# zongh5a/MDF-Net

Hardware: AMD Instinct MI355X
Metric: views/sec at DTU 1600x1200x5-view x4-scale (higher is better)
Workload: dtype f32; 1 GPU; DTU eval 1600x1184 (1600x1200 cropped as load/dtueval.py:34), 5 views, 3 cost-volume stages + x2 refine = 4 output scales, hypotheses (48,24,8), batch 1 per rank, seeded random weights (pth/dtu_29.pth is not available offline); parallelism=views sharded over 1 rank(s), no collective

## Files before the change

### mdf-net_amd/csrc/wino2d.hip

```cpp
#include <cstdlib>
#include <type_traits>
#include "common.h"
#include "conv_lds_common.h"
#define W3_PINNED_TILES_32
#include "wino3d_acc.h"

namespace {

template <int I, int N, typename F>
__device__ __forceinline__ void static_for(F&& f) {
  if constexpr (I < N) {
    f(std::integral_constant<int, I>{});
    static_for<I + 1, N>(f);
  }
}

struct Wino2dParams {
  const float* x;
  const float* wpack;
  const float* alpha;
  const float* beta;
  const float* res;
  float* y;
  float res_scale;
  int B, H, W, relu;
  int tiles_h, tiles_w, n_tiles;
};

template <int CIN, int COUT>
struct W2 {
  static_assert(CIN % 16 == 0 && COUT % 16 == 0 && COUT <= 64, "2-D Winograd form: Cin, Cout multiples of 16, Cout <= 64");
  static constexpr int NCH = CIN / 16, NT = COUT / 16, NG = CIN / 4;
  static constexpr int WN = (CIN >= 64) ? 2 : 1, NTW = NT / WN, WM = 4 / WN;
  static_assert(NT % WN == 0 && NTW >= 1 && NTW <= 2, "cout tiles per wave");
  static constexpr int TH = 2 * WM, TWO = 32;
  static constexpr int PH = TH + 2, PW = TWO + 2;
  static constexpr int NPP = PH * PW;
  static constexpr int S = round_s(NPP, 4, 2);
  static constexpr int PLANE = CIN * S;
  static constexpr int RING = 3;
  static constexpr int NPOS = NG * NPP;
  static constexpr int NFILL = (NPOS + 255) / 256;
  static constexpr int EPI_OFF = RING * PLANE;
  static constexpr int FRAG = 64 * 4;
  static constexpr int NSTEP = NCH * 16;
  static constexpr bool WL = ((size_t)(RING * PLANE + 128 + NSTEP * NT * FRAG) * sizeof(float) <= 160 * 1024);
  static constexpr int W_OFF = EPI_OFF + 128;
  static constexpr size_t LDS_BYTES = (size_t)(RING * PLANE + 128 + (WL ? NSTEP * NT * FRAG : 0)) * sizeof(float);
  static_assert(S > NPP, "a pad vector per group takes the fill's surplus lanes");
};

#ifndef MDF_W2_DIAG
#define MDF_W2_DIAG 0
#endif
#ifndef MDF_W2_HOLD_REL
#define MDF_W2_HOLD_REL 0
#endif
#ifndef MDF_W2_NA
#define MDF_W2_NA 4
#endif
#ifndef MDF_W2_WRITE_AB
#define MDF_W2_WRITE_AB 2
#endif

template <int CIN, int COUT, int NA, int WRITE_AB, bool S2D>
__global__ __launch_bounds__(256, 1) void wino2d_kernel(const Wino2dParams p) {
  typedef W2<CIN, COUT> C;
  constexpr int NCH = C::NCH, NT = C::NT, S = C::S, PW = C::PW, NPP = C::NPP, NFILL = C::NFILL, NSTEP = C::NSTEP;
  constexpr int AH = NA - 1;
  static_assert(NSTEP % NA == 0, "the fragment ring must close over a tile");
  extern __shared__ __attribute__((aligned(16))) float lds[];

  const int tid = threadIdx.x, lane = tid & 63;
  const int wave = __builtin_amdgcn_readfirstlane(tid >> 6);
  const int q = lane >> 4, n16 = lane & 15;
  const __amdgpu_buffer_rsrc_t wres = make_rsrc(p.wpack, (unsigned)(NSTEP * NT * 64 * 4 * 4));
  const int wvoff = lane * 16;
  const int wm = wave / C::WN, wn = wave % C::WN;
  constexpr int NTW = C::NTW;
  const int lane_lds = (q * S + wm * 2 * PW + n16 * 2) * 4;

  if (tid < 128) {
    const int c = tid & 63;
    lds[C::EPI_OFF + tid] = (tid < 64) ? ((c < COUT && p.alpha) ? p.alpha[c] : 1.f) : ((c < COUT && p.beta) ? p.beta[c] : 0.f);
  }
  if constexpr (C::WL) {
    constexpr int NV = NSTEP * NT * 64;
    for (int v = tid; v < NV; v += 256)
      *reinterpret_cast<float4*>(lds + C::W_OFF + v * 4) = *reinterpret_cast<const float4*>(p.wpack + (size_t)v * 4);
  }

  constexpr bool HOLD_REL = (NFILL <= 11) || (NTW == 1) || MDF_W2_HOLD_REL;
  constexpr int CM = S2D ? CIN / 4 : CIN;
  [[maybe_unused]] constexpr int GPP = CM / 4;
  auto rel_of = [&](int row, int col, int g) -> int {
    if constexpr (S2D) {
      const int par = g / GPP, c4 = g - par * GPP;
      return (((2 * row + (par >> 1)) * (2 * p.W) + 2 * col + (par & 1)) * CM + c4 * 4) * 4;
    } else {
      return ((row * p.W + col) * CIN + g * 4) * 4;
    }
  };
  int f_lds[NFILL], f_rc[NFILL], f_rel[HOLD_REL ? NFILL : 1];
#pragma unroll
  for (int k = 0; k < NFILL; ++k) {
    const int idx = tid + k * 256;
    const int glo = idx & 3, r = idx >> 2;
    const int v = r % NPP, g = (r / NPP) * 4 + glo;
    const bool live = idx < C::NPOS;
    const int row = live ? v / PW : 0x40, col = v % PW;
    f_lds[k] = live ? (g * S + v) * 4 : NPP * 4;
    f_rc[k] = (row << 16) | (col << 8) | g;
    if constexpr (HOLD_REL) f_rel[k] = live ? rel_of(row, col, g) : (int)0x80000000u;
  }

  const unsigned lb = mdf::xcd_remap(blockIdx.x, gridDim.x);
  const int t_begin = __builtin_amdgcn_readfirstlane((int)((unsigned long long)lb * (unsigned)p.n_tiles / gridDim.x));
  const int t_end = __builtin_amdgcn_readfirstlane((int)((unsigned long long)(lb + 1) * (unsigned)p.n_tiles / gridDim.x));
  if (t_begin >= t_end) return;

  float4 pf[NFILL];
  struct TileAt { int b, th, tw; };
  auto tile_at = [&](int t) -> TileAt {
    const int tw = t % p.tiles_w, rest = t / p.tiles_w;
    return TileAt{__builtin_amdgcn_readfirstlane(rest / p.tiles_h), __builtin_amdgcn_readfirstlane(rest % p.tiles_h), __builtin_amdgcn_readfirstlane(tw)};
  };
  auto tile_advance = [&](TileAt& c) {
    if (++c.tw == p.tiles_w) {
      c.tw = 0;
      if (++c.th == p.tiles_h) { c.th = 0; ++c.b; }
    }
  };
  auto issue_tile = [&](const TileAt& at, bool valid) {
    const int b = valid ? at.b : 0, h0 = (valid ? at.th : 0) * C::TH, w0 = (valid ? at.tw : 0) * C::TWO;
    const long long org = S2D ? ((long long)b * (2 * p.H) + 2 * (h0 - 1)) * (2 * p.W) + 2 * (w0 - 1)
                              : ((long long)b * p.H + (h0 - 1)) * p.W + (w0 - 1);
    const float* pz = p.x + org * CM;
    const unsigned long long pa = (unsigned long long)pz;
    const unsigned lo = (unsigned)__builtin_amdgcn_readfirstlane((int)(unsigned)pa), hi = (unsigned)__builtin_amdgcn_readfirstlane((int)(unsigned)(pa >> 32));
    const unsigned nrec = (!valid || (MDF_W2_DIAG & 1)) ? 0u : 0x7fffffffu;
    const __amdgpu_buffer_rsrc_t xr = make_rsrc((const void*)(((unsigned long long)hi << 32) | lo), nrec);
    const int r_lo = 1 - h0, r_hi = p.H + 1 - h0, c_lo = 1 - w0, c_hi = p.W + 1 - w0;
    if constexpr (HOLD_REL) {
      if (r_lo <= 0 && r_hi >= C::PH && c_lo <= 0 && c_hi >= C::PW) {
#pragma unroll
        for (int k = 0; k < NFILL; ++k) {
          const u32x4_t v = __builtin_amdgcn_raw_buffer_load_b128(xr, f_rel[k], 0, 0);
          pf[k] = make_float4(__uint_as_float(v.x), __uint_as_float(v.y), __uint_as_float(v.z), __uint_as_float(v.w));
        }
        return;
      }
    }
#pragma unroll
    for (int k = 0; k < NFILL; ++k) {
      const int row = f_rc[k] >> 16, col = (f_rc[k] >> 8) & 0xff;
      const bool ok = row >= r_lo && row < r_hi && col >= c_lo && col < c_hi;
      int rel;
      if constexpr (HOLD_REL) rel = f_rel[k];
      else rel = rel_of(row, col, f_rc[k] & 0xff);
      const u32x4_t v = __builtin_amdgcn_raw_buffer_load_b128(xr, ok ? rel : (int)0x80000000u, 0, 0);
      pf[k] = make_float4(__uint_as_float(v.x), __uint_as_float(v.y), __uint_as_float(v.z), __uint_as_float(v.w));
    }
  };
  auto write_tile = [&](int slot) {
#pragma unroll
    for (int k = 0; k < NFILL; ++k) *reinterpret_cast<float4*>(lds + slot * C::PLANE + f_lds[k]) = pf[k];
  };

  f32x2_t V[16][2], Dn[16][2];
  auto read_elem = [&](int slot, int ch, int e) {
    const int i = e >> 2, j = e & 3;
    float t[4];
    lds_frag<4>(lds + slot * C::PLANE + lane_lds + ((ch * 4) * S + i * PW + j) * 4, t);
    Dn[e][0] = (f32x2_t){t[0], t[1]};
    Dn[e][1] = (f32x2_t){t[2], t[3]};
  };
  auto transform = [&]() {
#pragma unroll
    for (int j = 0; j < 4; ++j)
#pragma unroll
      for (int c = 0; c < 2; ++c) {
        const f32x2_t d0 = Dn[j][c], d1 = Dn[4 + j][c], d2 = Dn[8 + j][c], d3 = Dn[12 + j][c];
        Dn[j][c] = d0 - d2; Dn[4 + j][c] = d1 + d2; Dn[8 + j][c] = d2 - d1; Dn[12 + j][c] = d1 - d3;
      }
#pragma unroll
    for (int a = 0; a < 4; ++a)
#pragma unroll
      for (int c = 0; c < 2; ++c) {
        const f32x2_t e0 = Dn[a * 4][c], e1 = Dn[a * 4 + 1][c], e2 = Dn[a * 4 + 2][c], e3 = Dn[a * 4 + 3][c];
        V[a * 4][c] = e0 - e2; V[a * 4 + 1][c] = e1 + e2; V[a * 4 + 2][c] = e2 - e1; V[a * 4 + 3][c] = e1 - e3;
      }
#pragma unroll
    for (int e = 0; e < 16; ++e)
#pragma unroll
      for (int c = 0; c < 2; ++c) asm volatile("" : "+v"(V[e][c]));
  };

  float af[NA][NTW][4];
  auto load_a = [&](int i, int buf) {
#pragma unroll
    for (int ntl = 0; ntl < NTW; ++ntl) {
      if constexpr (C::WL) lds_frag<4>(lds + C::W_OFF + (i * NT + wn * NTW + ntl) * C::FRAG + lane * 4, af[buf][ntl]);
      else buf_load_to<4>(wres, wvoff, (i * NT + wn * NTW + ntl) * (64 * 4 * 4), af[buf][ntl]);
    }
  };

  auto epilogue = [&](const TileAt& at) {
    const int b = at.b, h0 = at.th * C::TH, w0 = at.tw * C::TWO;
    if (h0 + 2 * wm >= p.H) return;
    const float* epi_tab = lds + C::EPI_OFF;
    asm volatile("s_nop 15\n\ts_nop 15" ::: "memory");
    static_for<0, NTW>([&](auto ntc) {
      constexpr int nt = decltype(ntc)::value;
      const int c0 = (wn * NTW + nt) * 16 + 4 * q;
      float yv[2][2][4];
      static_for<0, 2>([&](auto k2c) {
        constexpr int k2 = decltype(k2c)::value;
        float m[16][2];
        static_for<0, 16>([&](auto abc) { AccTile<nt * 16 + decltype(abc)::value>::template read2<k2>(m[decltype(abc)::value]); });
        f32x2_t srow[2][4];
#pragma unroll
        for (int bb = 0; bb < 4; ++bb) {
          const f32x2_t m0 = {m[bb][0], m[bb][1]}, m1 = {m[4 + bb][0], m[4 + bb][1]};
          const f32x2_t m2 = {m[8 + bb][0], m[8 + bb][1]}, m3 = {m[12 + bb][0], m[12 + bb][1]};
          srow[0][bb] = m0 + m1 + m2;
          srow[1][bb] = m1 - m2 - m3;
        }
#pragma unroll
        for (int pr = 0; pr < 2; ++pr) {
          const f32x2_t y0 = srow[pr][0] + srow[pr][1] + srow[pr][2];
          const f32x2_t y1 = srow[pr][1] - srow[pr][2] - srow[pr][3];
          yv[pr][0][2 * k2] = y0[0]; yv[pr][0][2 * k2 + 1] = y0[1];
          yv[pr][1][2 * k2] = y1[0]; yv[pr][1][2 * k2 + 1] = y1[1];
        }
      });
      float al_l[4], be_l[4];
#pragma unroll
      for (int k = 0; k < 4; ++k) { al_l[k] = epi_tab[c0 + k]; be_l[k] = epi_tab[64 + c0 + k]; }
#pragma unroll
      for (int pr = 0; pr < 2; ++pr) {
        const int h = h0 + 2 * wm + pr;
        if (h >= p.H) continue;
        const size_t row_vox = ((size_t)b * p.H + h) * p.W;
#pragma unroll
        for (int rr = 0; rr < 2; ++rr) {
          const int ow = w0 + 2 * n16 + rr;
          if (ow >= p.W) continue;
          float ov[4];
#pragma unroll
          for (int k = 0; k < 4; ++k) {
            ov[k] = yv[pr][rr][k] * al_l[k] + be_l[k];
            if (p.relu) ov[k] = fmaxf(ov[k], 0.f);
          }
          const size_t oi = (row_vox + ow) * COUT + c0;
          if (p.res) {
            const float4 rv = *reinterpret_cast<const float4*>(p.res + oi);
            ov[0] = rv.x + ov[0] * p.res_scale; ov[1] = rv.y + ov[1] * p.res_scale;
            ov[2] = rv.z + ov[2] * p.res_scale; ov[3] = rv.w + ov[3] * p.res_scale;
          }
          if (!(MDF_W2_DIAG & 2) || ov[0] == 1234.5f) *reinterpret_cast<float4*>(p.y + oi) = make_float4(ov[0], ov[1], ov[2], ov[3]);
        }
      }
    });
  };

  auto step = [&](auto rc, const TileAt& at, const TileAt& at_next2, bool valid_next2, bool has_next) {
    constexpr int R = decltype(rc)::value;
    constexpr int SLOT_N = (R + 1) % 3;
    static_for<0, NSTEP>([&](auto ic) {
      constexpr int i = decltype(ic)::value;
      constexpr int ch = i / 16, ab = i % 16;
      constexpr bool last_chunk = (ch == NCH - 1);
      if (!(MDF_W2_DIAG & 16)) load_a((i + AH) % NSTEP, (i + AH) % NA);
      if constexpr (ch == 0 && ab == WRITE_AB) {
        if (has_next) {
          write_tile(SLOT_N);
          __syncthreads();
        }
      }
      if constexpr (ab > WRITE_AB && ab <= WRITE_AB + 8 && !(MDF_W2_DIAG & 32)) {
        constexpr int e0 = 2 * (ab - WRITE_AB - 1);
        if constexpr (!last_chunk) { read_elem(R, ch + 1, e0); read_elem(R, ch + 1, e0 + 1); }
        else { read_elem(SLOT_N, 0, e0); read_elem(SLOT_N, 0, e0 + 1); }
      }
      __builtin_amdgcn_sched_barrier(0);
      static_for<0, NTW>([&](auto ntc) {
        constexpr int nt = decltype(ntc)::value;
        constexpr int T = nt * 16 + ab;
        if constexpr (ch == 0) AccTile<T>::mfma_fresh(af[i % NA][nt][0], V[ab][0][0]);
        else AccTile<T>::mfma(af[i % NA][nt][0], V[ab][0][0]);
        AccTile<T>::mfma(af[i % NA][nt][1], V[ab][0][1]);
        AccTile<T>::mfma(af[i % NA][nt][2], V[ab][1][0]);
        AccTile<T>::mfma(af[i % NA][nt][3], V[ab][1][1]);
      });
      __builtin_amdgcn_sched_barrier(0);
      if constexpr (ab == 15 && !last_chunk) { if (!(MDF_W2_DIAG & 8)) transform(); }
    });
    issue_tile(at_next2, valid_next2);
    if (!(MDF_W2_DIAG & 8)) transform();
    if (!(MDF_W2_DIAG & 4)) epilogue(at);
  };

  int t = t_begin;
  const int t_last = t_end - 1;
  TileAt at = tile_at(t), at2 = at;
  issue_tile(at, true);
  write_tile(0);
  __syncthreads();
  tile_advance(at2);
  issue_tile(at2, t < t_last);
  tile_advance(at2);
#pragma unroll
  for (int e = 0; e < 16; ++e) read_elem(0, 0, e);
  transform();
#pragma unroll
  for (int i = 0; i < AH; ++i) load_a(i, i % NA);

#define W2_STEP(RR)                                                                        \
  {                                                                                        \
    const bool has_next = t < t_last;                                                      \
    step(std::integral_constant<int, RR>{}, at, at2, t + 2 <= t_last, has_next);           \
    if (!has_next) break;                                                                  \
    ++t; tile_advance(at); tile_advance(at2);                                              \
  }
  for (;;) {
    W2_STEP(0)
    W2_STEP(1)
    W2_STEP(2)
  }
#undef W2_STEP
}

template <int CIN, int COUT, bool S2D = false>
int launch_wino2d(Wino2dParams& p, hipStream_t st) {
  typedef W2<CIN, COUT> C;
  constexpr int NA = MDF_W2_NA, WRITE_AB = MDF_W2_WRITE_AB;
  p.tiles_h = (p.H + C::TH - 1) / C::TH;
  p.tiles_w = (p.W + C::TWO - 1) / C::TWO;
  const long long tiles = (long long)p.B * p.tiles_h * p.tiles_w;
  if (tiles >= (1ll << 31)) return MDF_EUNSUPPORTED;
  p.n_tiles = (int)tiles;
  auto kern = &wino2d_kernel<CIN, COUT, NA, WRITE_AB, S2D>;
  static bool attr_done_dev[64] = {};
  int dev_id = 0;
  (void)hipGetDevice(&dev_id);
  bool& attr_done = attr_done_dev[(dev_id >= 0 && dev_id < 64) ? dev_id : 0];
  if (!attr_done || dev_id >= 64) {
    hipError_t e = hipFuncSetAttribute(reinterpret_cast<const void*>(kern), hipFuncAttributeMaxDynamicSharedMemorySize, (int)C::LDS_BYTES);
    if (e != hipSuccess) return mdf::fail(MDF_EHIP, "hipFuncSetAttribute(dynamic LDS %zu): %s", (size_t)C::LDS_BYTES, hipGetErrorString(e));
    attr_done = true;
  }
  long long grid = 256;
  if (const char* g = getenv("MDF_WINO2D_GRID")) { if (atoi(g) > 0) grid = atoi(g); }
  if (grid > tiles / 2) grid = tiles / 2;
  if (grid < 1) grid = 1;
  hipLaunchKernelGGL(kern, dim3((unsigned)grid), dim3(256), C::LDS_BYTES, st, p);
  return mdf::check_launch("wino2d_kernel");
}

}

int mdf_wino2d_dispatch(const float* x, const float* wpack_wino, const float* alpha, const float* beta, const float* res, float res_scale,
                        float* y, int B, int H, int W, int Cin, int Cout, int relu, void* stream) {
  Wino2dParams p{};
  p.x = x; p.wpack = wpack_wino; p.alpha = alpha; p.beta = beta; p.res = res; p.res_scale = res_scale; p.y = y;
  p.B = B; p.H = H; p.W = W; p.relu = relu;
  if ((long long)B * H * W * Cin * 4 >= (1ll << 31)) return MDF_EUNSUPPORTED;
  if (Cin == 16 && Cout == 16 && getenv("MDF_WINO2D_16")) return launch_wino2d<16, 16>(p, (hipStream_t)stream);
  if (Cin == 32 && Cout == 32) return launch_wino2d<32, 32>(p, (hipStream_t)stream);
  if (Cin == 64 && Cout == 64) return launch_wino2d<64, 64>(p, (hipStream_t)stream);
  return MDF_EUNSUPPORTED;
}

int mdf_wino2d_s2d_dispatch(const float* x, const float* wpack_k5w, const float* alpha, const float* beta, float* y, int B, int Ho, int Wo,
                            int Cin_mem, int Cout, int relu, void* stream) {
  Wino2dParams p{};
  p.x = x; p.wpack = wpack_k5w; p.alpha = alpha; p.beta = beta; p.res = nullptr; p.res_scale = 0.f; p.y = y;
  p.B = B; p.H = Ho; p.W = Wo; p.relu = relu;
  if ((long long)B * Ho * Wo * 4 * Cin_mem * 4 >= (1ll << 31)) return MDF_EUNSUPPORTED;
  if (Cin_mem == 16 && Cout == 32) return launch_wino2d<64, 32, true>(p, (hipStream_t)stream);
  if (Cin_mem == 8 && Cout == 16) return launch_wino2d<32, 16, true>(p, (hipStream_t)stream);
  return MDF_EUNSUPPORTED;
}
```

### mdf-net_amd/csrc/wino3d.hip

```cpp
#include <cstdlib>
#include <type_traits>
#include "common.h"
#include "conv_lds_common.h"
#include "wino3d_acc.h"

namespace {

template <int I, int N, typename F>
__device__ __forceinline__ void static_for(F&& f) {
  if constexpr (I < N) {
    f(std::integral_constant<int, I>{});
    static_for<I + 1, N>(f);
  }
}

struct Wino3dParams {
  const float* x;
  const float* wpack;
  const float* alpha;
  const float* beta;
  const float* res;
  float* y;
  float res_scale;
  int B, D, H, W, relu;
  int tiles_h, tiles_w;
  long long total;
};

template <int CIN, int COUT>
struct W3 {
  static_assert(CIN % 16 == 0 && COUT % 16 == 0 && COUT <= 64, "Winograd 3-D form: Cin, Cout multiples of 16");
  static constexpr int NCH = CIN / 16, NT = COUT / 16, NG = CIN / 4;
  static constexpr int WM = 4 / NT;
  static constexpr int TH = 2 * WM, TWO = 32;
  static constexpr int PH = TH + 2, PW = TWO + 2;
  static constexpr int NPP = PH * PW;
  static constexpr int S = round_s(NPP, 4, 2);
  static constexpr int PLANE = CIN * S;
  static constexpr int RING = 3;
  static constexpr int NPOS = NG * NPP;
  static constexpr int NFILL = (NPOS + 255) / 256;
  static constexpr int EPI_OFF = RING * PLANE;
  static constexpr int FRAG = 64 * 4;
  static constexpr int WL = ((size_t)(RING * PLANE + 128 + 3 * NCH * 16 * NT * FRAG) * sizeof(float) <= 160 * 1024) ? 3 : 0;
  static constexpr int W_OFF = EPI_OFF + 128;
  static constexpr size_t LDS_BYTES = (size_t)(RING * PLANE + 128 + WL * NCH * 16 * NT * FRAG) * sizeof(float);
  static_assert(S > NPP, "a pad vector per group takes the fill's surplus lanes");
};

#ifndef MDF_W3_DIAG
#define MDF_W3_DIAG 0
#endif
#ifndef MDF_W3_NOMASK
#define MDF_W3_NOMASK 0
#endif
#ifndef MDF_W3_PF_AT_START
#define MDF_W3_PF_AT_START 0
#endif
#ifndef MDF_W3_NA
#define MDF_W3_NA 4
#endif
#ifndef MDF_W3_WRITE_AB
#define MDF_W3_WRITE_AB 2
#endif
template <int CIN, int COUT, int NA, int WRITE_AB>
__global__ __launch_bounds__(256, 1) void wino3d_kernel(const Wino3dParams p) {
  typedef W3<CIN, COUT> C;
  constexpr int NCH = C::NCH, NT = C::NT, S = C::S, PW = C::PW, NPP = C::NPP, NFILL = C::NFILL;
  constexpr int AH = NA - 1;
  constexpr int NSTEP = NCH * 16;
  static_assert(NSTEP % NA == 0, "the fragment ring must close over a plane");
  extern __shared__ __attribute__((aligned(16))) float lds[];

  const int tid = threadIdx.x, lane = tid & 63;
  const int wave = __builtin_amdgcn_readfirstlane(tid >> 6);
  const int q = lane >> 4, n16 = lane & 15;
  const int wm = wave / NT, wn = wave % NT;
  const __amdgpu_buffer_rsrc_t wres = make_rsrc(p.wpack, (unsigned)(3 * NCH * 16 * NT * 64 * 4 * 4));
  const int wvoff = lane * 16;
  const int lane_lds = (q * S + wm * 2 * PW + n16 * 2) * 4;

  if (tid < 128) {
    const int c = tid & 63;
    lds[C::EPI_OFF + tid] = (tid < 64) ? ((c < COUT && p.alpha) ? p.alpha[c] : 1.f) : ((c < COUT && p.beta) ? p.beta[c] : 0.f);
  }

  if constexpr (C::WL > 0) {
    constexpr int NV = C::WL * NSTEP * NT * 64;
    for (int v = tid; v < NV; v += 256)
      *reinterpret_cast<float4*>(lds + C::W_OFF + v * 4) = *reinterpret_cast<const float4*>(p.wpack + (size_t)v * 4);
  }

  int f_lds[NFILL];
#pragma unroll
  for (int k = 0; k < NFILL; ++k) {
    const int idx = tid + k * 256;
    const int glo = idx & 3, r = idx >> 2;
    const int v = r % NPP, ghi = r / NPP;
    f_lds[k] = (idx < C::NPOS) ? ((ghi * 4 + glo) * S + v) * 4 : NPP * 4;
  }

  const size_t plane_elems = (size_t)p.H * p.W * CIN;
  const unsigned plane_bytes = (unsigned)(plane_elems * 4);

  const unsigned lb = mdf::xcd_remap(blockIdx.x, gridDim.x);
  unsigned s_cur = (unsigned)((unsigned long long)lb * (unsigned)p.total / gridDim.x);
  const unsigned s_end = (unsigned)((unsigned long long)(lb + 1) * (unsigned)p.total / gridDim.x);

  while (s_cur < s_end) {
    const int tile_l = __builtin_amdgcn_readfirstlane((int)(s_cur / (unsigned)p.D));
    const int da = __builtin_amdgcn_readfirstlane((int)(s_cur - (unsigned)tile_l * (unsigned)p.D));
    const int db = __builtin_amdgcn_readfirstlane((int)min((unsigned)p.D, (unsigned)da + (s_end - s_cur)));
    s_cur += db - da;
    const int tw = __builtin_amdgcn_readfirstlane(tile_l % p.tiles_w);
    const int th = __builtin_amdgcn_readfirstlane((tile_l / p.tiles_w) % p.tiles_h);
    const int b = __builtin_amdgcn_readfirstlane(tile_l / (p.tiles_w * p.tiles_h));
    const int h0 = th * C::TH, w0 = tw * C::TWO;
    const bool wave_live = (h0 + 2 * wm) < p.H;

    unsigned f_off[NFILL];
    {
      int tid_l = tid;
      asm volatile("" : "+v"(tid_l));
#pragma unroll
      for (int k = 0; k < NFILL; ++k) {
        const int idx = tid_l + k * 256;
        const int glo = idx & 3, r2 = idx >> 2;
        const int v = r2 % NPP, g = (r2 / NPP) * 4 + glo;
        const int ih = h0 - 1 + v / PW, iw = w0 - 1 + v % PW;
        const bool ok = idx < C::NPOS && ih >= 0 && ih < p.H && iw >= 0 && iw < p.W;
        f_off[k] = ok ? (unsigned)(((ih * p.W + iw) * CIN + g * 4) * 4) : 0x80000000u;
      }
    }
    const float* xb = p.x + (size_t)b * p.D * plane_elems;
    float4 pf[NFILL];
    auto issue_plane = [&](int z) {
      const bool in = z >= 0 && z < p.D;
      const float* pz = xb + (size_t)(in ? z : 0) * plane_elems;
      const unsigned long long pa = (unsigned long long)pz;
      const unsigned lo = (unsigned)__builtin_amdgcn_readfirstlane((int)(unsigned)pa), hi = (unsigned)__builtin_amdgcn_readfirstlane((int)(unsigned)(pa >> 32));
      const unsigned nrec = (MDF_W3_DIAG & 1) ? 0u : (unsigned)__builtin_amdgcn_readfirstlane((int)(in ? plane_bytes : 0u));
      const __amdgpu_buffer_rsrc_t xr = make_rsrc((const void*)(((unsigned long long)hi << 32) | lo), nrec);
#pragma unroll
      for (int k = 0; k < NFILL; ++k) {
        const u32x4_t v = __builtin_amdgcn_raw_buffer_load_b128(xr, (int)f_off[k], 0, 0);
        pf[k] = make_float4(__uint_as_float(v.x), __uint_as_float(v.y), __uint_as_float(v.z), __uint_as_float(v.w));
      }
    };
    auto write_plane = [&](int slot) {
#pragma unroll
      for (int k = 0; k < NFILL; ++k) *reinterpret_cast<float4*>(lds + slot * C::PLANE + f_lds[k]) = pf[k];
    };

    f32x2_t V[16][2];
    f32x2_t Dn[16][2];
    auto read_elem = [&](int slot, int ch, int e) {
      const int i = e >> 2, j = e & 3;
      float t[4];
      lds_frag<4>(lds + slot * C::PLANE + lane_lds + ((ch * 4) * S + i * PW + j) * 4, t);
      Dn[e][0] = (f32x2_t){t[0], t[1]};
      Dn[e][1] = (f32x2_t){t[2], t[3]};
    };
    auto transform = [&]() {
#pragma unroll
      for (int j = 0; j < 4; ++j)
#pragma unroll
        for (int c = 0; c < 2; ++c) {
          const f32x2_t d0 = Dn[j][c], d1 = Dn[4 + j][c], d2 = Dn[8 + j][c], d3 = Dn[12 + j][c];
          Dn[j][c] = d0 - d2; Dn[4 + j][c] = d1 + d2; Dn[8 + j][c] = d2 - d1; Dn[12 + j][c] = d1 - d3;
        }
#pragma unroll
      for (int a = 0; a < 4; ++a)
#pragma unroll
        for (int c = 0; c < 2; ++c) {
          const f32x2_t e0 = Dn[a * 4][c], e1 = Dn[a * 4 + 1][c], e2 = Dn[a * 4 + 2][c], e3 = Dn[a * 4 + 3][c];
          V[a * 4][c] = e0 - e2; V[a * 4 + 1][c] = e1 + e2; V[a * 4 + 2][c] = e2 - e1; V[a * 4 + 3][c] = e1 - e3;
        }
#pragma unroll
      for (int e = 0; e < 16; ++e)
#pragma unroll
        for (int c = 0; c < 2; ++c) asm volatile("" : "+v"(V[e][c]));
    };

    float af[NA][3][4];
    auto load_a = [&](int i, int buf) {
#pragma unroll
      for (int kd = 0; kd < 3; ++kd) {
        if (kd < C::WL) lds_frag<4>(lds + C::W_OFF + ((kd * NSTEP + i) * NT + wn) * C::FRAG + lane * 4, af[buf][kd]);
        else buf_load_to<4>(wres, wvoff, ((kd * NSTEP + i) * NT + wn) * (64 * 4 * 4), af[buf][kd]);
      }
    };

    auto epilogue = [&](auto setc, int o) {
      constexpr int SET = decltype(setc)::value;
      if (!wave_live) return;
      const float* epi_tab = lds + C::EPI_OFF;
      const int c0 = wn * 16 + 4 * q;
      asm volatile("s_nop 15\n\ts_nop 15" ::: "memory");
      float yv[2][2][4];
      static_for<0, 2>([&](auto k2c) {
        constexpr int k2 = decltype(k2c)::value;
        float m[16][2];
        static_for<0, 16>([&](auto abc) { AccTile<SET * 16 + decltype(abc)::value>::template read2<k2>(m[decltype(abc)::value]); });
        f32x2_t srow[2][4];
#pragma unroll
        for (int bb = 0; bb < 4; ++bb) {
          const f32x2_t m0 = {m[bb][0], m[bb][1]}, m1 = {m[4 + bb][0], m[4 + bb][1]};
          const f32x2_t m2 = {m[8 + bb][0], m[8 + bb][1]}, m3 = {m[12 + bb][0], m[12 + bb][1]};
          srow[0][bb] = m0 + m1 + m2;
          srow[1][bb] = m1 - m2 - m3;
        }
#pragma unroll
        for (int pr = 0; pr < 2; ++pr) {
          const f32x2_t y0 = srow[pr][0] + srow[pr][1] + srow[pr][2];
          const f32x2_t y1 = srow[pr][1] - srow[pr][2] - srow[pr][3];
          yv[pr][0][2 * k2] = y0[0]; yv[pr][0][2 * k2 + 1] = y0[1];
          yv[pr][1][2 * k2] = y1[0]; yv[pr][1][2 * k2 + 1] = y1[1];
        }
      });
      float al_l[4], be_l[4];
#pragma unroll
      for (int k = 0; k < 4; ++k) { al_l[k] = epi_tab[c0 + k]; be_l[k] = epi_tab[64 + c0 + k]; }
#pragma unroll
      for (int pr = 0; pr < 2; ++pr) {
        const int h = h0 + 2 * wm + pr;
        if (h >= p.H) continue;
        const size_t row_vox = (((size_t)b * p.D + o) * p.H + h) * p.W;
#pragma unroll
        for (int rr = 0; rr < 2; ++rr) {
          const int ow = w0 + 2 * n16 + rr;
          if (ow >= p.W) continue;
          float ov[4];
#pragma unroll
          for (int k = 0; k < 4; ++k) {
            ov[k] = yv[pr][rr][k] * al_l[k] + be_l[k];
            if (p.relu) ov[k] = fmaxf(ov[k], 0.f);
          }
          const size_t oi = (row_vox + ow) * COUT + c0;
          if (p.res) {
            const float4 rv = *reinterpret_cast<const float4*>(p.res + oi);
            ov[0] = rv.x + ov[0] * p.res_scale; ov[1] = rv.y + ov[1] * p.res_scale;
            ov[2] = rv.z + ov[2] * p.res_scale; ov[3] = rv.w + ov[3] * p.res_scale;
          }
          if (!(MDF_W3_DIAG & 2) || ov[0] == 1234.5f) *reinterpret_cast<float4*>(p.y + oi) = make_float4(ov[0], ov[1], ov[2], ov[3]);
        }
      }
    };

    auto step = [&](auto rc, int zi, int z_next2, bool has_next, bool k0, bool k1, bool k2, bool fresh1) {
      constexpr int R = decltype(rc)::value;
      const bool all3 = MDF_W3_NOMASK || (k0 && k1 && k2 && !fresh1);
      if (MDF_W3_PF_AT_START) issue_plane(has_next ? zi + 1 : -1);
      constexpr int SLOT_N = (R + 1) % 3;
      static_for<0, NSTEP>([&](auto ic) {
        constexpr int i = decltype(ic)::value;
        constexpr int ch = i / 16, ab = i % 16;
        constexpr bool last_chunk = (ch == NCH - 1);
        if (!(MDF_W3_DIAG & 16)) load_a((i + AH) % NSTEP, (i + AH) % NA);
        if constexpr (ch == 0 && ab == WRITE_AB) {
          if (has_next) {
            write_plane(SLOT_N);
            __syncthreads();
          }
        }
        if constexpr (ab > WRITE_AB && ab <= WRITE_AB + 8) {
          constexpr int e0 = 2 * (ab - WRITE_AB - 1);
          if constexpr (!last_chunk) { read_elem(R, ch + 1, e0); read_elem(R, ch + 1, e0 + 1); }
          else { read_elem(SLOT_N, 0, e0); read_elem(SLOT_N, 0, e0 + 1); }
        }
        __builtin_amdgcn_sched_barrier(0);
        constexpr int S0 = ((R + 1) % 3) * 16 + ab, S1 = R * 16 + ab, S2 = ((R + 2) % 3) * 16 + ab;
        if (__builtin_expect(all3, 1)) {
          if constexpr (ch == 0) AccTile<S0>::mfma_fresh(af[i % NA][0][0], V[ab][0][0]);
          else AccTile<S0>::mfma(af[i % NA][0][0], V[ab][0][0]);
          AccTile<S0>::mfma(af[i % NA][0][1], V[ab][0][1]);
          AccTile<S0>::mfma(af[i % NA][0][2], V[ab][1][0]);
          AccTile<S0>::mfma(af[i % NA][0][3], V[ab][1][1]);
          AccTile<S1>::mfma(af[i % NA][1][0], V[ab][0][0]);
          AccTile<S1>::mfma(af[i % NA][1][1], V[ab][0][1]);
          AccTile<S1>::mfma(af[i % NA][1][2], V[ab][1][0]);
          AccTile<S1>::mfma(af[i % NA][1][3], V[ab][1][1]);
          AccTile<S2>::mfma(af[i % NA][2][0], V[ab][0][0]);
          AccTile<S2>::mfma(af[i % NA][2][1], V[ab][0][1]);
          AccTile<S2>::mfma(af[i % NA][2][2], V[ab][1][0]);
          AccTile<S2>::mfma(af[i % NA][2][3], V[ab][1][1]);
        } else {
          if (k0) {
            if constexpr (ch == 0) AccTile<S0>::mfma_fresh(af[i % NA][0][0], V[ab][0][0]);
            else AccTile<S0>::mfma(af[i % NA][0][0], V[ab][0][0]);
            AccTile<S0>::mfma(af[i % NA][0][1], V[ab][0][1]);
            AccTile<S0>::mfma(af[i % NA][0][2], V[ab][1][0]);
            AccTile<S0>::mfma(af[i % NA][0][3], V[ab][1][1]);
          }
          if (k1) {
            if constexpr (ch == 0) {
              if (fresh1) AccTile<S1>::mfma_fresh(af[i % NA][1][0], V[ab][0][0]);
              else AccTile<S1>::mfma(af[i % NA][1][0], V[ab][0][0]);
            } else {
              AccTile<S1>::mfma(af[i % NA][1][0], V[ab][0][0]);
            }
            AccTile<S1>::mfma(af[i % NA][1][1], V[ab][0][1]);
            AccTile<S1>::mfma(af[i % NA][1][2], V[ab][1][0]);
            AccTile<S1>::mfma(af[i % NA][1][3], V[ab][1][1]);
          }
          if (k2) {
            AccTile<S2>::mfma(af[i % NA][2][0], V[ab][0][0]);
            AccTile<S2>::mfma(af[i % NA][2][1], V[ab][0][1]);
            AccTile<S2>::mfma(af[i % NA][2][2], V[ab][1][0]);
            AccTile<S2>::mfma(af[i % NA][2][3], V[ab][1][1]);
          }
        }
        __builtin_amdgcn_sched_barrier(0);
        if constexpr (ab == 15 && !last_chunk) { if (!(MDF_W3_DIAG & 8)) transform(); }
      });
      if (!MDF_W3_PF_AT_START) issue_plane(z_next2);
      if (!(MDF_W3_DIAG & 8)) transform();
      if (k2 && !(MDF_W3_DIAG & 4)) epilogue(std::integral_constant<int, (R + 2) % 3>{}, zi - 1);
    };

    int zi = (da == 0) ? 0 : da - 1;
    const int z_last = (db == p.D) ? p.D - 1 : db;
    __syncthreads();
    issue_plane(zi);
    write_plane(0);
    __syncthreads();
    if (!MDF_W3_PF_AT_START) issue_plane(zi < z_last ? zi + 1 : -1);
#pragma unroll
    for (int e = 0; e < 16; ++e) read_elem(0, 0, e);
    transform();
#pragma unroll
    for (int i = 0; i < AH; ++i) load_a(i, i % NA);

    int r_last = 0;
#define W3_STEP(RR)                                                                                          \
    {                                                                                                        \
      const bool has_next = zi < z_last;                                                                     \
      step(std::integral_constant<int, RR>{}, zi, (zi + 2 <= z_last) ? zi + 2 : -1, has_next,                \
           zi + 1 >= da && zi + 1 < db, zi >= da && zi < db, zi - 1 >= da && zi - 1 < db, zi == 0);          \
      if (!has_next) { r_last = RR; break; }                                                                 \
      ++zi;                                                                                                  \
    }
    for (;;) {
      W3_STEP(0)
      W3_STEP(1)
      W3_STEP(2)
    }
#undef W3_STEP
    if (db == p.D) {
      switch (r_last) {
        case 0: epilogue(std::integral_constant<int, 0>{}, p.D - 1); break;
        case 1: epilogue(std::integral_constant<int, 1>{}, p.D - 1); break;
        default: epilogue(std::integral_constant<int, 2>{}, p.D - 1); break;
      }
    }
  }
}

template <int CIN, int COUT>
int launch_wino3d(Wino3dParams& p, hipStream_t st) {
  typedef W3<CIN, COUT> C;
  constexpr int NA = MDF_W3_NA;
  constexpr int WRITE_AB = MDF_W3_WRITE_AB;
  p.tiles_h = (p.H + C::TH - 1) / C::TH;
  p.tiles_w = (p.W + C::TWO - 1) / C::TWO;
  p.total = (long long)p.B * p.tiles_h * p.tiles_w * p.D;
  if (p.total >= (1ll << 31)) return MDF_EUNSUPPORTED;
  auto kern = &wino3d_kernel<CIN, COUT, NA, WRITE_AB>;
  static bool attr_done_dev[64] = {};
  int dev_id = 0;
  (void)hipGetDevice(&dev_id);
  bool& attr_done = attr_done_dev[(dev_id >= 0 && dev_id < 64) ? dev_id : 0];
  if (!attr_done || dev_id >= 64) {
    hipError_t e = hipFuncSetAttribute(reinterpret_cast<const void*>(kern), hipFuncAttributeMaxDynamicSharedMemorySize, (int)C::LDS_BYTES);
    if (e != hipSuccess) return mdf::fail(MDF_EHIP, "hipFuncSetAttribute(dynamic LDS %zu): %s", (size_t)C::LDS_BYTES, hipGetErrorString(e));
    attr_done = true;
  }
  long long grid = 256;
  if (const char* g = getenv("MDF_WINO3D_GRID")) { if (atoi(g) > 0) grid = atoi(g); }
  if (grid > p.total / 4) grid = p.total / 4;
  if (grid < 1) grid = 1;
  hipLaunchKernelGGL(kern, dim3((unsigned)grid), dim3(256), C::LDS_BYTES, st, p);
  return mdf::check_launch("wino3d_kernel");
}

}

int mdf_wino3d_dispatch(const float* x, const float* wpack_wino, const float* alpha, const float* beta, const float* res, float res_scale,
                        float* y, int B, int D, int H, int W, int Cin, int Cout, int relu, void* stream) {
  Wino3dParams p{};
  p.x = x; p.wpack = wpack_wino; p.alpha = alpha; p.beta = beta; p.res = res; p.res_scale = res_scale; p.y = y;
  p.B = B; p.D = D; p.H = H; p.W = W; p.relu = relu;
  if ((long long)H * W * Cin * 4 >= (1ll << 31)) return MDF_EUNSUPPORTED;
  if (Cin == 32 && Cout == 16) return launch_wino3d<32, 16>(p, (hipStream_t)stream);
  if (Cin == 16 && Cout == 16) return launch_wino3d<16, 16>(p, (hipStream_t)stream);
  return MDF_EUNSUPPORTED;
}
```

Before: 297.8 views/s.

## Cover ragged right-edge columns with tall narrow Winograd strip tiles

Result: no change. 298.5 views/s, median of 6 (+0.3%).

```diff
diff --git a/mdf-net_amd/csrc/wino2d.hip b/mdf-net_amd/csrc/wino2d.hip
--- a/mdf-net_amd/csrc/wino2d.hip
+++ b/mdf-net_amd/csrc/wino2d.hip
@@ -4,6 +4,7 @@
 #include "conv_lds_common.h"
 #define W3_PINNED_TILES_32
 #include "wino3d_acc.h"
+#include "wino_tile_plan.h"
 
 namespace {
 
@@ -24,7 +25,8 @@
   float* y;
   float res_scale;
   int B, H, W, relu;
-  int tiles_h, tiles_w, n_tiles;
+  WinoTilePlan plan;
+  int n_tiles;
 };
 
 template <int CIN, int COUT>
@@ -78,7 +80,8 @@
   const int wvoff = lane * 16;
   const int wm = wave / C::WN, wn = wave % C::WN;
   constexpr int NTW = C::NTW;
-  const int lane_lds = (q * S + wm * 2 * PW + n16 * 2) * 4;
+  static_assert(C::TH == 2 * C::WM && (C::TH == 8 || C::TH == 4), "wino_tile_plan.h: the 8-row and the 4-row family");
+  const int mcol = wm * 16 + n16;
 
   if (tid < 128) {
     const int c = tid & 63;
@@ -107,12 +110,34 @@
     const int idx = tid + k * 256;
     const int glo = idx & 3, r = idx >> 2;
     const int v = r % NPP, g = (r / NPP) * 4 + glo;
-    const bool live = idx < C::NPOS;
-    const int row = live ? v / PW : 0x40, col = v % PW;
-    f_lds[k] = live ? (g * S + v) * 4 : NPP * 4;
-    f_rc[k] = (row << 16) | (col << 8) | g;
-    if constexpr (HOLD_REL) f_rel[k] = live ? rel_of(row, col, g) : (int)0x80000000u;
-  }
+    f_lds[k] = (idx < C::NPOS) ? (g * S + v) * 4 : NPP * 4;
+  }
+  int g_fill = -1;
+  auto set_fill_geom = [&](int geom) {
+    const int gpw = wino_tile_geom(C::TH, geom).pw, gph = wino_tile_geom(C::TH, geom).th + 2;
+    int tid_l = tid;
+    asm volatile("" : "+v"(tid_l));
+#pragma unroll
+    for (int k = 0; k < NFILL; ++k) {
+      const int idx = tid_l + k * 256;
+      const int glo = idx & 3, r = idx >> 2;
+      const int v = r % NPP, g = (r / NPP) * 4 + glo;
+      const int prow = (geom == 0) ? v / PW : (geom == 1) ? v / 10 : v / 18, col = v - prow * gpw;
+      const bool live = idx < C::NPOS && prow < gph;
+      const int row = live ? prow : 0x40;
+      f_rc[k] = (row << 16) | (col << 8) | g;
+      if constexpr (HOLD_REL) f_rel[k] = live ? rel_of(row, col, g) : (int)0x80000000u;
+    }
+    g_fill = geom;
+  };
+  int row_lds[4], g_read = -1;
+  auto set_read_geom = [&](int geom) {
+    const WinoTileGeom gg = wino_tile_geom(C::TH, geom);
+    const int rp = mcol >> gg.shift, wt = mcol & ((1 << gg.shift) - 1);
+#pragma unroll
+    for (int i = 0; i < 4; ++i) row_lds[i] = (q * S + (rp * 2 + i) * gg.pw + wt * 2) * 4;
+    g_read = geom;
+  };
 
   const unsigned lb = mdf::xcd_remap(blockIdx.x, gridDim.x);
   const int t_begin = __builtin_amdgcn_readfirstlane((int)((unsigned long long)lb * (unsigned)p.n_tiles / gridDim.x));
@@ -120,19 +145,31 @@
   if (t_begin >= t_end) return;
 
   float4 pf[NFILL];
-  struct TileAt { int b, th, tw; };
+  struct TileAt { int b, r, h0, w0, geom; };
+  const int n_main = p.plan.main_h * p.plan.main_w, w_main = p.plan.main_w * C::TWO, strip_th = wino_tile_geom(C::TH, p.plan.geom).th;
   auto tile_at = [&](int t) -> TileAt {
-    const int tw = t % p.tiles_w, rest = t / p.tiles_w;
-    return TileAt{__builtin_amdgcn_readfirstlane(rest / p.tiles_h), __builtin_amdgcn_readfirstlane(rest % p.tiles_h), __builtin_amdgcn_readfirstlane(tw)};
+    const int b = t / p.plan.per_img, r = t - b * p.plan.per_img;
+    const WinoTile tl = wino_tile_at(p.plan, C::TH, r);
+    return TileAt{__builtin_amdgcn_readfirstlane(b), __builtin_amdgcn_readfirstlane(r), __builtin_amdgcn_readfirstlane(tl.h0),
+                  __builtin_amdgcn_readfirstlane(tl.w0), __builtin_amdgcn_readfirstlane(tl.geom)};
   };
   auto tile_advance = [&](TileAt& c) {
-    if (++c.tw == p.tiles_w) {
-      c.tw = 0;
-      if (++c.th == p.tiles_h) { c.th = 0; ++c.b; }
+    if (++c.r == p.plan.per_img) { c.r = 0; ++c.b; }
+    if (c.r == 0 || c.r == n_main) {
+      c.geom = (c.r < n_main) ? 0 : p.plan.geom;
+      c.h0 = 0;
+      c.w0 = (c.r < n_main) ? 0 : w_main;
+    } else if (c.r < n_main) {
+      c.w0 += C::TWO;
+      if (c.w0 == w_main) { c.w0 = 0; c.h0 += C::TH; }
+    } else {
+      c.h0 += strip_th;
     }
   };
   auto issue_tile = [&](const TileAt& at, bool valid) {
-    const int b = valid ? at.b : 0, h0 = (valid ? at.th : 0) * C::TH, w0 = (valid ? at.tw : 0) * C::TWO;
+    const int b = valid ? at.b : 0, h0 = valid ? at.h0 : 0, w0 = valid ? at.w0 : 0;
+    if (valid && at.geom != g_fill) set_fill_geom(at.geom);
+    const int gph = wino_tile_geom(C::TH, g_fill).th + 2, gpw = wino_tile_geom(C::TH, g_fill).pw;
     const long long org = S2D ? ((long long)b * (2 * p.H) + 2 * (h0 - 1)) * (2 * p.W) + 2 * (w0 - 1)
                               : ((long long)b * p.H + (h0 - 1)) * p.W + (w0 - 1);
     const float* pz = p.x + org * CM;
@@ -142,7 +179,7 @@
     const __amdgpu_buffer_rsrc_t xr = make_rsrc((const void*)(((unsigned long long)hi << 32) | lo), nrec);
     const int r_lo = 1 - h0, r_hi = p.H + 1 - h0, c_lo = 1 - w0, c_hi = p.W + 1 - w0;
     if constexpr (HOLD_REL) {
-      if (r_lo <= 0 && r_hi >= C::PH && c_lo <= 0 && c_hi >= C::PW) {
+      if (r_lo <= 0 && r_hi >= gph && c_lo <= 0 && c_hi >= gpw) {
 #pragma unroll
         for (int k = 0; k < NFILL; ++k) {
           const u32x4_t v = __builtin_amdgcn_raw_buffer_load_b128(xr, f_rel[k], 0, 0);
@@ -171,7 +208,7 @@
   auto read_elem = [&](int slot, int ch, int e) {
     const int i = e >> 2, j = e & 3;
     float t[4];
-    lds_frag<4>(lds + slot * C::PLANE + lane_lds + ((ch * 4) * S + i * PW + j) * 4, t);
+    lds_frag<4>(lds + slot * C::PLANE + row_lds[i] + ((ch * 4) * S + j) * 4, t);
     Dn[e][0] = (f32x2_t){t[0], t[1]};
     Dn[e][1] = (f32x2_t){t[2], t[3]};
   };
@@ -206,8 +243,10 @@
   };
 
   auto epilogue = [&](const TileAt& at) {
-    const int b = at.b, h0 = at.th * C::TH, w0 = at.tw * C::TWO;
-    if (h0 + 2 * wm >= p.H) return;
+    const int b = at.b, h0 = at.h0, w0 = at.w0;
+    const int gsh = wino_tile_geom(C::TH, at.geom).shift;
+    if (h0 + 2 * ((wm * 16) >> gsh) >= p.H) return;
+    const int rp = mcol >> gsh, wt = mcol & ((1 << gsh) - 1);
     const float* epi_tab = lds + C::EPI_OFF;
     asm volatile("s_nop 15\n\ts_nop 15" ::: "memory");
     static_for<0, NTW>([&](auto ntc) {
@@ -239,12 +278,12 @@
       for (int k = 0; k < 4; ++k) { al_l[k] = epi_tab[c0 + k]; be_l[k] = epi_tab[64 + c0 + k]; }
 #pragma unroll
       for (int pr = 0; pr < 2; ++pr) {
-        const int h = h0 + 2 * wm + pr;
+        const int h = h0 + 2 * rp + pr;
         if (h >= p.H) continue;
         const size_t row_vox = ((size_t)b * p.H + h) * p.W;
 #pragma unroll
         for (int rr = 0; rr < 2; ++rr) {
-          const int ow = w0 + 2 * n16 + rr;
+          const int ow = w0 + 2 * wt + rr;
           if (ow >= p.W) continue;
           float ov[4];
 #pragma unroll
@@ -267,6 +306,8 @@
   auto step = [&](auto rc, const TileAt& at, const TileAt& at_next2, bool valid_next2, bool has_next) {
     constexpr int R = decltype(rc)::value;
     constexpr int SLOT_N = (R + 1) % 3;
+    TileAt at_next = at;
+    tile_advance(at_next);
     static_for<0, NSTEP>([&](auto ic) {
       constexpr int i = decltype(ic)::value;
       constexpr int ch = i / 16, ab = i % 16;
@@ -278,6 +319,7 @@
           __syncthreads();
         }
       }
+      if constexpr (last_chunk && ab == WRITE_AB) { if (has_next && at_next.geom != g_read) set_read_geom(at_next.geom); }
       if constexpr (ab > WRITE_AB && ab <= WRITE_AB + 8 && !(MDF_W2_DIAG & 32)) {
         constexpr int e0 = 2 * (ab - WRITE_AB - 1);
         if constexpr (!last_chunk) { read_elem(R, ch + 1, e0); read_elem(R, ch + 1, e0 + 1); }
@@ -304,6 +346,7 @@
   int t = t_begin;
   const int t_last = t_end - 1;
   TileAt at = tile_at(t), at2 = at;
+  set_read_geom(at.geom);
   issue_tile(at, true);
   write_tile(0);
   __syncthreads();
@@ -335,9 +378,8 @@
 int launch_wino2d(Wino2dParams& p, hipStream_t st) {
   typedef W2<CIN, COUT> C;
   constexpr int NA = MDF_W2_NA, WRITE_AB = MDF_W2_WRITE_AB;
-  p.tiles_h = (p.H + C::TH - 1) / C::TH;
-  p.tiles_w = (p.W + C::TWO - 1) / C::TWO;
-  const long long tiles = (long long)p.B * p.tiles_h * p.tiles_w;
+  p.plan = wino_tile_plan(p.H, p.W, C::TH, wino_strips_enabled());
+  const long long tiles = (long long)p.B * p.plan.per_img;
   if (tiles >= (1ll << 31)) return MDF_EUNSUPPORTED;
   p.n_tiles = (int)tiles;
   auto kern = &wino2d_kernel<CIN, COUT, NA, WRITE_AB, S2D>;
diff --git a/mdf-net_amd/csrc/wino3d.hip b/mdf-net_amd/csrc/wino3d.hip
--- a/mdf-net_amd/csrc/wino3d.hip
+++ b/mdf-net_amd/csrc/wino3d.hip
@@ -3,6 +3,7 @@
 #include "common.h"
 #include "conv_lds_common.h"
 #include "wino3d_acc.h"
+#include "wino_tile_plan.h"
 
 namespace {
 
@@ -23,7 +24,7 @@
   float* y;
   float res_scale;
   int B, D, H, W, relu;
-  int tiles_h, tiles_w;
+  WinoTilePlan plan;
   long long total;
 };
 
@@ -78,7 +79,8 @@
   const int wm = wave / NT, wn = wave % NT;
   const __amdgpu_buffer_rsrc_t wres = make_rsrc(p.wpack, (unsigned)(3 * NCH * 16 * NT * 64 * 4 * 4));
   const int wvoff = lane * 16;
-  const int lane_lds = (q * S + wm * 2 * PW + n16 * 2) * 4;
+  static_assert(C::WM == 4 && C::TH == 8, "wino_tile_plan.h: the 8-row family");
+  const int mcol = wm * 16 + n16;
 
   if (tid < 128) {
     const int c = tid & 63;
@@ -112,11 +114,17 @@
     const int da = __builtin_amdgcn_readfirstlane((int)(s_cur - (unsigned)tile_l * (unsigned)p.D));
     const int db = __builtin_amdgcn_readfirstlane((int)min((unsigned)p.D, (unsigned)da + (s_end - s_cur)));
     s_cur += db - da;
-    const int tw = __builtin_amdgcn_readfirstlane(tile_l % p.tiles_w);
-    const int th = __builtin_amdgcn_readfirstlane((tile_l / p.tiles_w) % p.tiles_h);
-    const int b = __builtin_amdgcn_readfirstlane(tile_l / (p.tiles_w * p.tiles_h));
-    const int h0 = th * C::TH, w0 = tw * C::TWO;
-    const bool wave_live = (h0 + 2 * wm) < p.H;
+    const int b = __builtin_amdgcn_readfirstlane(tile_l / p.plan.per_img);
+    const WinoTile tl = wino_tile_at(p.plan, C::TH, tile_l - b * p.plan.per_img);
+    const int h0 = __builtin_amdgcn_readfirstlane(tl.h0), w0 = __builtin_amdgcn_readfirstlane(tl.w0);
+    const int geom = __builtin_amdgcn_readfirstlane(tl.geom);
+    const int gsh = (geom == 0) ? 4 : (geom == 1) ? 2 : 3;
+    const int gpw = (geom == 0) ? PW : (geom == 1) ? 10 : 18, gph = (geom == 0) ? C::PH : (geom == 1) ? 34 : 18;
+    const int rp = mcol >> gsh, wt = mcol & ((1 << gsh) - 1);
+    const bool wave_live = (h0 + 2 * ((wm * 16) >> gsh)) < p.H;
+    int row_lds[4];
+#pragma unroll
+    for (int i = 0; i < 4; ++i) row_lds[i] = (q * S + (rp * 2 + i) * gpw + wt * 2) * 4;
 
     unsigned f_off[NFILL];
     {
@@ -127,8 +135,9 @@
         const int idx = tid_l + k * 256;
         const int glo = idx & 3, r2 = idx >> 2;
         const int v = r2 % NPP, g = (r2 / NPP) * 4 + glo;
-        const int ih = h0 - 1 + v / PW, iw = w0 - 1 + v % PW;
-        const bool ok = idx < C::NPOS && ih >= 0 && ih < p.H && iw >= 0 && iw < p.W;
+        const int prow = (geom == 0) ? v / PW : (geom == 1) ? v / 10 : v / 18, pcol = v - prow * gpw;
+        const int ih = h0 - 1 + prow, iw = w0 - 1 + pcol;
+        const bool ok = idx < C::NPOS && prow < gph && ih >= 0 && ih < p.H && iw >= 0 && iw < p.W;
         f_off[k] = ok ? (unsigned)(((ih * p.W + iw) * CIN + g * 4) * 4) : 0x80000000u;
       }
     }
@@ -157,7 +166,7 @@
     auto read_elem = [&](int slot, int ch, int e) {
       const int i = e >> 2, j = e & 3;
       float t[4];
-      lds_frag<4>(lds + slot * C::PLANE + lane_lds + ((ch * 4) * S + i * PW + j) * 4, t);
+      lds_frag<4>(lds + slot * C::PLANE + row_lds[i] + ((ch * 4) * S + j) * 4, t);
       Dn[e][0] = (f32x2_t){t[0], t[1]};
       Dn[e][1] = (f32x2_t){t[2], t[3]};
     };
@@ -223,12 +232,12 @@
       for (int k = 0; k < 4; ++k) { al_l[k] = epi_tab[c0 + k]; be_l[k] = epi_tab[64 + c0 + k]; }
 #pragma unroll
       for (int pr = 0; pr < 2; ++pr) {
-        const int h = h0 + 2 * wm + pr;
+        const int h = h0 + 2 * rp + pr;
         if (h >= p.H) continue;
         const size_t row_vox = (((size_t)b * p.D + o) * p.H + h) * p.W;
 #pragma unroll
         for (int rr = 0; rr < 2; ++rr) {
-          const int ow = w0 + 2 * n16 + rr;
+          const int ow = w0 + 2 * wt + rr;
           if (ow >= p.W) continue;
           float ov[4];
 #pragma unroll
@@ -361,9 +370,8 @@
   typedef W3<CIN, COUT> C;
   constexpr int NA = MDF_W3_NA;
   constexpr int WRITE_AB = MDF_W3_WRITE_AB;
-  p.tiles_h = (p.H + C::TH - 1) / C::TH;
-  p.tiles_w = (p.W + C::TWO - 1) / C::TWO;
-  p.total = (long long)p.B * p.tiles_h * p.tiles_w * p.D;
+  p.plan = wino_tile_plan(p.H, p.W, C::TH, wino_strips_enabled());
+  p.total = (long long)p.B * p.plan.per_img * p.D;
   if (p.total >= (1ll << 31)) return MDF_EUNSUPPORTED;
   auto kern = &wino3d_kernel<CIN, COUT, NA, WRITE_AB>;
   static bool attr_done_dev[64] = {};
diff --git a/mdf-net_amd/csrc/wino_tile_plan.h b/mdf-net_amd/csrc/wino_tile_plan.h
--- /dev/null
+++ b/mdf-net_amd/csrc/wino_tile_plan.h
@@ -0,0 +1,71 @@
+#pragma once
+#include <cstdlib>
+
+#if defined(__HIPCC__)
+#define WINO_PLAN_HD __host__ __device__ __forceinline__
+#else
+#define WINO_PLAN_HD inline
+#endif
+
+struct WinoTilePlan {
+  int main_h;
+  int main_w;
+  int strip_n;
+  int geom;
+  int per_img;
+};
+
+struct WinoTileGeom {
+  int th, tw;
+  int pw;
+  int shift;
+};
+
+struct WinoTile {
+  int h0, w0;
+  int geom;
+};
+
+constexpr int WINO_MAIN_TW = 32;
+
+WINO_PLAN_HD WinoTileGeom wino_tile_geom(int th_main, int geom) {
+  const int cols = 8 * th_main;
+  if (geom == 1) return WinoTileGeom{2 * (cols >> 2), 8, 10, 2};
+  if (geom == 2) return WinoTileGeom{2 * (cols >> 3), 16, 18, 3};
+  return WinoTileGeom{th_main, WINO_MAIN_TW, WINO_MAIN_TW + 2, 4};
+}
+
+WINO_PLAN_HD WinoTilePlan wino_tile_plan(int H, int W, int th_main, bool strips) {
+  WinoTilePlan pl;
+  pl.main_h = (H + th_main - 1) / th_main;
+  pl.main_w = (W + WINO_MAIN_TW - 1) / WINO_MAIN_TW;
+  pl.strip_n = 0;
+  pl.geom = 0;
+  const int rem = W % WINO_MAIN_TW;
+  if (strips && rem >= 1 && rem <= 16) {
+    const int g = rem <= 8 ? 1 : 2;
+    const int sth = wino_tile_geom(th_main, g).th;
+    const int sn = (H + sth - 1) / sth;
+    if (sn < pl.main_h) {
+      pl.main_w = W / WINO_MAIN_TW;
+      pl.strip_n = sn;
+      pl.geom = g;
+    }
+  }
+  pl.per_img = pl.main_h * pl.main_w + pl.strip_n;
+  return pl;
+}
+
+WINO_PLAN_HD WinoTile wino_tile_at(const WinoTilePlan& pl, int th_main, int r) {
+  const int n_main = pl.main_h * pl.main_w;
+  if (r < n_main) {
+    const int th = r / pl.main_w;
+    return WinoTile{th * th_main, (r - th * pl.main_w) * WINO_MAIN_TW, 0};
+  }
+  return WinoTile{(r - n_main) * wino_tile_geom(th_main, pl.geom).th, pl.main_w * WINO_MAIN_TW, pl.geom};
+}
+
+inline bool wino_strips_enabled() {
+  const char* e = getenv("MDF_WINO_STRIPS");
+  return e ? atoi(e) != 0 : true;
+}
```
